# tjuDavidWang/MARL-UAVs-Targets-Tracking

Measured on AMD Instinct MI355X. Metric: env agent-steps/sec, higher is better.
Workload: dtype f32

## Files before the change

### marl-uavs-targets-tracking_amd/csrc/greedy.h

```cpp
#pragma once
#include "env.h"
#include "philox.h"

namespace uavtrack {

template <typename UPos>
__device__ __forceinline__ int greedy_near_count(float2 t, int N, float dc2, UPos upos)
{
    int c = 0;
    for (int j = 0; j < N; ++j) {
        const float2 u = upos(j);
        c += (fmaf(u.y - t.y, u.y - t.y, (u.x - t.x) * (u.x - t.x)) < dc2) ? 1 : 0;
    }
    return c;
}

template <typename UPos, typename TPos, typename Near>
__device__ __forceinline__ int greedy_pick(float x, float y, float h, int i, int N, int M, int na, float dc2,
                                           float turn_unit, uint64_t genv, uint32_t step, uint32_t k0, uint32_t k1,
                                           UPos upos, TPos tpos, Near near)
{
    const Philox4 r = philox4x32_10((uint32_t)genv, step, (uint32_t)i, 0x47524459u ^ (uint32_t)(genv >> 32), k0, k1);
    if (u01(r.v[0]) < 0.25f)
        return (int)(((uint64_t)r.v[1] * (uint32_t)na) >> 32);
    int same = 0;
    for (int j = 0; j < N; ++j) {
        const float2 u = upos(j);
        same += (u.x == x && u.y == y) ? 1 : 0;
    }
    float best = -INFINITY, best_dx = 1.0f, best_dy = 0.0f;
    for (int k = 0; k < M; ++k) {
        const float2 t = tpos(k);
        const float dx = t.x - x, dy = t.y - y;
        const float d2 = fmaf(dy, dy, dx * dx);
        const int others = near(k) - (d2 < dc2 ? same : 0);
        const float score = __builtin_amdgcn_rsqf(d2) - 0.8f * (float)others;
        if (score > best) { best = score; best_dx = dx; best_dy = dy; }
    }
    float angle = atan2f(best_dy, best_dx) - h;
    if (u01(r.v[2]) < 0.3f) angle = 0.0f;
    angle -= kTwoPi * floorf((angle + kPi) * (1.0f / kTwoPi));
    int besta = 0;
    float bestd = INFINITY;
    for (int a = 0; a < na; ++a) {
        const float dd = fabsf(angle - (float)(2 * a + 1 - na) * turn_unit);
        if (dd < bestd) { bestd = dd; besta = a; }
    }
    return besta;
}

}
```

### marl-uavs-targets-tracking_amd/csrc/step_kernel.hip

```cpp

#include "actor.h"
#include "greedy.h"
#include "philox.h"

#include <cstdlib>

#define UAVTRACK_UNROLL_U 5
#define UAVTRACK_UNROLL_T 5

namespace uavtrack {

namespace {

typedef float v2f __attribute__((ext_vector_type(2)));

struct Acc {
    float cntU, iwU, sxU, syU, scU, ssU, saU;
    float cntT, iwT, sxT, syT, scT, ssT;
    float trk;
    float dup;
};

constexpr int kLoneActorTiles = 4;
constexpr float kSymMagic = 12582912.0f;
// ... 92 lines not shown

template <typename T>
__device__ __forceinline__ T *at(T *base, unsigned byte_off)
{
    return (T *)((char *)base + byte_off);
}

typedef unsigned v2u_nt __attribute__((ext_vector_type(2)));
template <typename T>
__device__ __forceinline__ void out_store(T *ptr, T v)
{
    __builtin_nontemporal_store(v, ptr);
}
__device__ __forceinline__ void out_store(uint2 *ptr, unsigned a, unsigned b)
{
    const v2u_nt q = {a, b};
    __builtin_nontemporal_store(q, reinterpret_cast<v2u_nt *>(ptr));
}

__device__ __host__ __forceinline__ int obs_stage_f4(int lanes) { return ((lanes + 63) / 64) * 192; }
__device__ __host__ __forceinline__ int pairs_of(int n) { return (n + 1) >> 1; }
constexpr int kCovPairs = 12;
__device__ __host__ __forceinline__ int cov_words(int m) { return (pairs_of(m) + kCovPairs - 1) / kCovPairs; }
__device__ __host__ __forceinline__ int ustride_of(int n)
{
    const int s = pairs_of(n) * 6;
    return (s * 4) % 64 == 0 ? s + 1 : s;
}
__device__ __host__ __forceinline__ int tstride_of(int m)
{
    const int s = pairs_of(m) * 2;
    return (s * 4) % 64 == 0 ? s + 1 : s;
}

__device__ __host__ __forceinline__ int sym_pose_len(int n) { return n + n / 2 + 1; }
__device__ __host__ __forceinline__ int sym_words(int n, bool z3) { return sym_pose_len(n) * (z3 ? 3 : 2) + 2 * n; }

struct UavRow { float x, y, c, s, a, z; };
__device__ __forceinline__ UavRow uav_elem(const float4 *rows, int j)
{
    const float *f = reinterpret_cast<const float *>(rows + (j >> 1) * 6);
    const int b = j & 1;
    return UavRow{f[b], f[2 + b], f[4 + b], f[6 + b], f[8 + b], f[10 + b]};
}
__device__ __forceinline__ void uav_store(float4 *rows, int j, float x, float y, float c, float s, float a, float z)
{
    float *f = reinterpret_cast<float *>(rows + (j >> 1) * 6);
    const int b = j & 1;
    f[b] = x; f[2 + b] = y; f[4 + b] = c; f[6 + b] = s; f[8 + b] = a; f[10 + b] = z;
}

__device__ __host__ constexpr bool act_bias_shape(int n_spec) { return n_spec > 0 && n_spec <= 64; }

template <int N_, int M_, bool Z3, bool NB, int PF, bool SYM = false, bool VC = false, bool NBSEQ = false>
__device__ __forceinline__ void sweep_fast(const StepParams &p, int N, int M, int i,
                                           const float4 *__restrict__ rowNew, const float4 *__restrict__ rowOld,
                                           const float4 *__restrict__ trow, const v2f *__restrict__ tzrow,
                                           unsigned *__restrict__ covw, int covbase,
                                           float xi, float yi, float zi, float ci, float si, float ai,
                                           float xo, float yo, float zo, float co, float so, float ao, Acc &a,
                                           unsigned long long &nbmask, const float4 *const *__restrict__ rsel = nullptr,
                                           const float4 *__restrict__ ubase = nullptr, unsigned copyw = 0)
{
    const v2f xi2 = splat(xi), yi2 = splat(yi), zi2 = splat(zi);
    const v2f nscale = splat(p.le_neg_scale);
    constexpr bool kActBias = act_bias_shape(N_);
    const int NP = pairs_of(N_ > 0 ? N_ : N), MP = pairs_of(M_ > 0 ? M_ : M);
    constexpr int UU = (N_ > 0 && (N_ + 1) / 2 <= 10) ? (N_ + 1) / 2 : UAVTRACK_UNROLL_U;

    v2f sx = splat(0.f), sy = splat(0.f), sc = splat(0.f), ss = splat(0.f), cnt = splat(0.f), trk = splat(0.f);
    v2f cov = splat(0.f);
    constexpr int QM = M_ > 0 ? (M_ + 1) / 2 : 1, QN = N_ > 0 ? (N_ + 1) / 2 : 1;
    constexpr bool kPrefetch = PF > 0 && N_ > 0 && M_ > 0 && QN <= 10 && QM <= 5 && !Z3;
    float4 Q0[QM], Q1[QM], PN0[QN], PM0[QN], PM1[QN];
    v2f PM2[QN];
    auto copy_row = [&](int jp) -> const float4 * {
        if constexpr (N_ > 0 && N_ <= 64)
            return reinterpret_cast<const float4 *>(reinterpret_cast<const char *>(ubase) + __builtin_amdgcn_ubfe(copyw, (unsigned)jp, 1u) * 48u);
        return (2 * jp < i) ? rowNew : rowOld;
    };
    auto fetch_row = [&](int jq) {
        const float4 *rq = rsel ? rsel[jq] : copy_row(jq);
        PN0[jq] = rowNew[jq * 6]; PM0[jq] = rq[jq * 6]; PM1[jq] = rq[jq * 6 + 1];
        PM2[jq] = *reinterpret_cast<const v2f *>(&rq[jq * 6 + 2]);
    };
    if (kPrefetch) {
#pragma unroll
        for (int kp = 0; kp < QM; ++kp) { Q0[kp] = trow[kp * 2]; Q1[kp] = trow[kp * 2 + 1]; }
#pragma unroll
        for (int jq = 0; jq < PF && jq < QN; ++jq) fetch_row(jq);
        __builtin_amdgcn_sched_barrier(0x407);
    }
    auto target_pair = [&](int kp) {
        const float4 q0 = kPrefetch ? Q0[kPrefetch ? kp : 0] : trow[kp * 2], q1 = kPrefetch ? Q1[kPrefetch ? kp : 0] : trow[kp * 2 + 1];
        const v2f dx = (v2f){q0.x, q0.y} - xi2, dy = (v2f){q0.z, q0.w} - yi2;
        v2f d2 = pk_fma(dy, dy, dx * dx);
        if (Z3) { const v2f dz = tzrow[kp] - zi2; d2 = pk_fma(dz, dz, d2); }
        const v2f dist = {fast_sqrt(d2.x), fast_sqrt(d2.y)};
        const v2f mm = pk_le_mask<VC>(d2, nscale, p.le_dp2);
        sx = pk_fma(mm, dx, sx);
        sy = pk_fma(mm, dy, sy);
        sc = pk_fma(mm, (v2f){q1.x, q1.y}, sc);
        ss = pk_fma(mm, (v2f){q1.z, q1.w}, ss);
        cnt += mm;
        trk = pk_fma(mm, dist, trk);
        cov = pk_fma(cov, splat(4.0f), pk_le_mask<VC>(d2, nscale, p.lt_dp2));
    };
    auto flush_word = [&](int w) {
        const unsigned bits = (unsigned)cov.x | ((unsigned)cov.y << 1);
        if (bits) atomicOr(&covw[covbase + w], bits);
        cov = splat(0.f);
    };
    if constexpr (M_ > 0) {
        constexpr int MPc = (M_ + 1) / 2, CWc = (MPc + kCovPairs - 1) / kCovPairs;
#pragma unroll
        for (int w = 0; w < CWc; ++w) {
            constexpr int kInner = MPc <= UAVTRACK_UNROLL_T ? MPc : 6;
            const int k1 = (w + 1) * kCovPairs < MPc ? (w + 1) * kCovPairs : MPc;
#pragma unroll kInner
            for (int kp = w * kCovPairs; kp < k1; ++kp) target_pair(kp);
            flush_word(w);
        }
    } else {
        for (int w = 0; w * kCovPairs < MP; ++w) {
            const int k1 = min((w + 1) * kCovPairs, MP);
#pragma unroll 4
            for (int kp = w * kCovPairs; kp < k1; ++kp) target_pair(kp);
            flush_word(w);
        }
    }
    a.cntT = cnt.x + cnt.y; a.iwT = a.cntT;
    a.sxT = sx.x + sx.y; a.syT = sy.x + sy.y; a.trk = fmaf(-(trk.x + trk.y), p.inv_dp, 2.0f * a.cntT);
    a.scT = fmaf(sc.x + sc.y, p.vratio, -ci * a.cntT);
    a.ssT = fmaf(ss.x + ss.y, p.vratio, -si * a.cntT);

    sx = splat(0.f); sy = splat(0.f); sc = splat(0.f); ss = splat(0.f); cnt = splat(0.f);
    v2f sa = splat(0.f), dup = splat(0.f);
    constexpr bool NBF = NB && N_ > 0 && (N_ + 1) / 2 <= kCovPairs;
    v2f nbf = splat(0.f);
    const float4 *ub = ubase;
#pragma unroll UU
    for (int jp = 0; jp < NP; ++jp) {
        const float4 *rp;
        if (rsel && kPrefetch) rp = rsel[kPrefetch ? jp : 0] + jp * 6;
        else if constexpr (N_ > 0 && N_ <= 64) rp = reinterpret_cast<const float4 *>(reinterpret_cast<const char *>(ub) + __builtin_amdgcn_ubfe(copyw, (unsigned)jp, 1u) * 48u);
        else rp = copy_row(jp) + jp * 6;
        ub += 6;
        if (kPrefetch) {
            if (jp + PF < NP) fetch_row(jp + PF);
            __builtin_amdgcn_sched_barrier(0x407);
        }
        const float4 n0 = kPrefetch ? PN0[kPrefetch ? jp : 0] : rowNew[jp * 6];
        const float4 m0 = kPrefetch ? PM0[kPrefetch ? jp : 0] : rp[0], m1 = kPrefetch ? PM1[kPrefetch ? jp : 0] : rp[1];
        const float4 m2 = kPrefetch ? make_float4(PM2[kPrefetch ? jp : 0].x, PM2[kPrefetch ? jp : 0].y, 0.f, 0.f) : rp[2];
        const v2f dxn = (v2f){n0.x, n0.y} - xi2, dyn = (v2f){n0.z, n0.w} - yi2;
        const v2f dxm = (v2f){m0.x, m0.y} - xi2, dym = (v2f){m0.z, m0.w} - yi2;
        v2f d2n = pk_fma(dyn, dyn, dxn * dxn), d2m = pk_fma(dym, dym, dxm * dxm);
        if (Z3) {
            const v2f dzm = (v2f){m2.z, m2.w} - zi2;
            d2m = pk_fma(dzm, dzm, d2m);
            if (!SYM || NB) {
                const float4 n2 = rowNew[jp * 6 + 2];
                const v2f dzn = (v2f){n2.z, n2.w} - zi2;
                d2n = pk_fma(dzn, dzn, d2n);
            }
        }
        if (NBF)
            nbf = pk_fma(nbf, splat(4.0f), pk_le_mask<VC>(NBSEQ ? d2m : d2n, nscale, p.le_dp2));
        else if (NB)
            nbmask |= ((unsigned long long)(d2n.x <= p.dp2 ? 1u : 0u) | (unsigned long long)(d2n.y <= p.dp2 ? 2u : 0u)) << (2 * jp);
        if (!SYM) {
            const v2f w = pk_fma((v2f){fast_sqrt(d2n.x), fast_sqrt(d2n.y)}, splat(-p.exp_k1), splat(p.exp_k0));
            dup = pk_fma(pk_le_mask<VC>(d2n, nscale, p.le_two_dp2), (v2f){fast_exp2(w.x), fast_exp2(w.y)}, dup);
        }
        const v2f mm = pk_le_mask<VC>(d2m, nscale, p.le_dc2);
        sx = pk_fma(mm, dxm, sx);
        sy = pk_fma(mm, dym, sy);
        sc = pk_fma(mm, (v2f){m1.x, m1.y}, sc);
        ss = pk_fma(mm, (v2f){m1.z, m1.w}, ss);
        sa = pk_fma(mm, (v2f){m2.x, m2.y}, sa);
        if (!kActBias) cnt += mm;
    }
    if (NBF) {
        const unsigned w = (unsigned)nbf.y | ((unsigned)nbf.x << 1);
        nbmask = (unsigned long long)(__brev(w) >> (32 - 2 * NP));
    }
    const bool odd = i & 1;
    const float dxs = xo - xi, dys = yo - yi;
    float d2s = dist2(dxs, dys);
    if (Z3) { const float dzs = zo - zi; d2s = fmaf(dzs, dzs, d2s); }
    const float mse = (!odd && d2s <= p.dc2) ? 1.0f : 0.0f;
    a.dup = dup.x + dup.y - fast_exp2(p.exp_k0);
    float cnt_all = cnt.x + cnt.y, sa_all = sa.x + sa.y;
    if (kActBias) {
        cnt_all = floorf(sa_all * p.inv_act_bias);
        sa_all = fmaf(-p.act_bias, cnt_all, sa_all);
    }
    a.cntU = cnt_all - (odd ? 1.0f : mse); a.iwU = a.cntU;
    a.sxU = fmaf(-mse, dxs, sx.x + sx.y);
    a.syU = fmaf(-mse, dys, sy.x + sy.y);
    a.scU = fmaf(-mse, co - ci, fmaf(-ci, cnt_all, sc.x + sc.y));
    a.ssU = fmaf(-mse, so - si, fmaf(-si, cnt_all, ss.x + ss.y));
    a.saU = fmaf(-mse, ao - ai, fmaf(-ai, cnt_all, sa_all));
}

template <int N_, bool Z3, bool VC = false>
__device__ __forceinline__ unsigned sym_dup(const StepParams &p, int N, int i, const float *__restrict__ sx, const float *__restrict__ sy,
                                            const float *__restrict__ sz, unsigned *__restrict__ dacc, float xi, float yi, float zi)
{
    const int n = N_ > 0 ? N_ : N;
    const int KP = (n - 1) / 2;
    const v2f xi2 = splat(xi), yi2 = splat(yi), zi2 = splat(zi), nscale = splat(p.le_neg_scale);
    unsigned own = 0;
    struct P2 { v2f x, y, z; };
    auto load2 = [&](int k) {
        P2 q;
        q.x = (v2f){sx[i + k], sx[i + k + 1]};
        q.y = (v2f){sy[i + k], sy[i + k + 1]};
        q.z = Z3 ? (v2f){sz[i + k], sz[i + k + 1]} : splat(0.f);
        return q;
    };
    auto eval2 = [&](const P2 &q) {
        const v2f dx = q.x - xi2, dy = q.y - yi2;
        v2f d2 = pk_fma(dy, dy, dx * dx);
        if (Z3) { const v2f dz = q.z - zi2; d2 = pk_fma(dz, dz, d2); }
        const v2f w = pk_fma((v2f){fast_sqrt(d2.x), fast_sqrt(d2.y)}, splat(-p.exp_k1), splat(p.sym_k0));
        const v2f g = pk_fma(pk_le_mask<VC>(d2, nscale, p.le_two_dp2), (v2f){fast_exp2(w.x), fast_exp2(w.y)}, splat(kSymMagic));
        return make_uint2(__float_as_uint(g.x), __float_as_uint(g.y));
    };
    constexpr int UK = (N_ > 0 && (N_ - 1) / 2 <= 10) ? 5 : 4;
    const int last = KP + ((n & 1) == 0 ? 1 : 0);
    P2 cur = load2(1);
#pragma unroll UK
    for (int k = 1; k + 1 <= KP; k += 2) {
        P2 nxt = cur;
        if (k + 2 <= last) nxt = load2(k + 2);
        const uint2 q = eval2(cur);
        own += q.x + q.y;
        atomicAdd(&dacc[i + k], q.x);
        atomicAdd(&dacc[i + k + 1], q.y);
        cur = nxt;
    }
    if (KP & 1) {
        const uint2 q = eval2(cur);
        own += q.x;
        atomicAdd(&dacc[i + KP], q.x);
        if ((n & 1) == 0) own += q.y;
    } else if ((n & 1) == 0) {
        const uint2 q = eval2(cur);
        own += q.x;
    }
    return own;
}

template <bool Z3>
__device__ __forceinline__ void sweep_weighted(const StepParams &p, int N, int M, int i,
                                               const float4 *__restrict__ rowNew, const float4 *__restrict__ rowOld,
                                               const float4 *__restrict__ trow, const v2f *__restrict__ tzrow,
                                               unsigned *__restrict__ covw, int covbase,
                                               float xi, float yi, float zi, float ci, float si, float ai, float abias, Acc &a)
{
    a = Acc{0, 0, 0, 0, 0, 0, 0, 0, 0, 0, 0, 0, 0, 0, 0};
    unsigned bits = 0;
#pragma unroll 1
    for (int k = 0; k < M; ++k) {
        const float *f = reinterpret_cast<const float *>(trow + (k >> 1) * 2);
        const int b = k & 1;
        const float dx = f[b] - xi, dy = f[2 + b] - yi, tc = f[4 + b], ts = f[6 + b];
        float d2 = dist2(dx, dy);
        if (Z3) { const float dz = reinterpret_cast<const float *>(tzrow)[k] - zi; d2 = fmaf(dz, dz, d2); }
        const float d = fast_sqrt(d2);
        const bool in = d2 <= p.dp2;
        const float m = in ? 1.0f : 0.0f;
        const float rx = dx * p.inv_dp - xi, ry = dy * p.inv_dp - yi;
        const float iw = in ? 1.0f / fminf(sqrtf(rx * rx + ry * ry), 1.0f) : 0.0f;
        a.scT = fmaf(iw, tc * p.vratio - ci, a.scT);
        a.ssT = fmaf(iw, ts * p.vratio - si, a.ssT);
        a.cntT += m;
        a.iwT += iw;
        a.sxT = fmaf(iw, dx, a.sxT);
        a.syT = fmaf(iw, dy, a.syT);
        a.trk = fmaf(m, fmaf(-d, p.inv_dp, 2.0f), a.trk);
        {
            const int kp = k >> 1, word = kp / kCovPairs, MPw = pairs_of(M);
            const int in_word = min(kCovPairs, MPw - word * kCovPairs);
            bits |= (d2 < p.dp2) ? (1u << (2 * (in_word - 1 - kp % kCovPairs) + (k & 1))) : 0u;
            if ((kp % kCovPairs == kCovPairs - 1 && (k & 1)) || k == M - 1) {
                if (bits) atomicOr(&covw[covbase + word], bits);
                bits = 0;
            }
        }
    }
#pragma unroll 1
    for (int j = 0; j < N; ++j) {
        const bool other = (j != i);
        const UavRow nw = uav_elem(rowNew, j);
        const UavRow mx = uav_elem((j < i) ? rowNew : rowOld, j);
        const float dxn = nw.x - xi, dyn = nw.y - yi, dxm = mx.x - xi, dym = mx.y - yi;
        float d2n = dist2(dxn, dyn), d2m = dist2(dxm, dym);
        if (Z3) {
            const float dzn = nw.z - zi, dzm = mx.z - zi;
            d2n = fmaf(dzn, dzn, d2n);
            d2m = fmaf(dzm, dzm, d2m);
        }
        const float ex = fast_exp2(fmaf(fast_sqrt(d2n), -p.exp_k1, p.exp_k0));
        a.dup += (other && d2n <= p.two_dp2) ? ex : 0.0f;
        const bool inm = other && d2m <= p.dc2;
        const float m = inm ? 1.0f : 0.0f;
        const float rx = dxm * p.inv_dc - xi, ry = dym * p.inv_dc - yi;
        const float iw = inm ? 1.0f / fminf(sqrtf(rx * rx + ry * ry), 1.0f) : 0.0f;
        a.scU = fmaf(iw, mx.c - ci, a.scU);
        a.ssU = fmaf(iw, mx.s - si, a.ssU);
        a.saU = fmaf(iw, (mx.a - abias) - ai, a.saU);
        a.cntU += m;
        a.iwU += iw;
        a.sxU = fmaf(iw, dxm, a.sxU);
        a.syU = fmaf(iw, dym, a.syU);
    }
}

template <int N_, int M_, int MODE, bool Z3, int POLICY, bool ALLOUT = false, bool EXTRAS = false, bool LONE = false>
__global__ void __launch_bounds__(kMaxWorkgroup) rollout_kernel(const StepParams p_in)
{
    constexpr bool kVConst = LONE;
    StepParams p = p_in;
    if (kVConst) {
#define UAVTRACK_V(f) p.f = vreg(p_in.f)
        UAVTRACK_V(inv_dp); UAVTRACK_V(inv_dc); UAVTRACK_V(dp2); UAVTRACK_V(dc2); UAVTRACK_V(dup_k); UAVTRACK_V(sym_dup_k);
        UAVTRACK_V(vratio); UAVTRACK_V(inv_na_total); UAVTRACK_V(exp_k0); UAVTRACK_V(exp_k1); UAVTRACK_V(x_max); UAVTRACK_V(y_max);
        UAVTRACK_V(tt_ceil); UAVTRACK_V(inv_tt_ceil); UAVTRACK_V(alpha); UAVTRACK_V(beta); UAVTRACK_V(gamma);
        UAVTRACK_V(sym_k0); UAVTRACK_V(act_bias); UAVTRACK_V(inv_act_bias);
        UAVTRACK_V(le_neg_scale); UAVTRACK_V(le_dp2); UAVTRACK_V(lt_dp2); UAVTRACK_V(le_dc2); UAVTRACK_V(le_two_dp2);
        UAVTRACK_V(dtv_u); UAVTRACK_V(dtv_t); UAVTRACK_V(turn_unit); UAVTRACK_V(inv_na); UAVTRACK_V(two_dp2); UAVTRACK_V(dp); UAVTRACK_V(coop);
#undef UAVTRACK_V
    }
    constexpr bool GREEDY = POLICY == kPolicyGreedy;
    constexpr bool ACTOR = POLICY == kPolicyActor;
    constexpr bool GIVEN = POLICY == kPolicyGiven;
    extern __shared__ float4 smem4[];
    if (ALLOUT) __builtin_assume(p.obs != nullptr && p.reward != nullptr && p.terms != nullptr && p.covered != nullptr && p.done != nullptr);
    if (POLICY == kPolicyGiven) __builtin_assume(p.actions != nullptr);
    const int N = N_ > 0 ? N_ : p.N;
    const int M = M_ > 0 ? M_ : p.M;
    const int E = p.E;
    const int EN = E * N;
    const int CW = cov_words(M);
    const int MP = pairs_of(M);
    const float abias = act_bias_shape(N_) ? p.act_bias : 0.0f;
    const int tid = threadIdx.x;
    const int nthreads = blockDim.x;
    using NbMask = typename NbMaskOf<N_>::type;
    constexpr int kNbBits = 8 * (int)sizeof(NbMask);

    const int ustride = ustride_of(N), tstride = tstride_of(M);
    float4 *utab = smem4;
    float4 *ttab = utab + E * ustride;
    float4 *ostg = ttab + E * tstride;
    float *fb = reinterpret_cast<float *>(ostg + obs_stage_f4(E * N));
    float *thd = fb;   fb += E * M;
// ... 47 lines not shown
            for (int w = 0; w < CW; ++w) covw[e * CW + w] = covw[E * CW + e * CW + w] = 0;
            if (M & 1) {
                float *f = reinterpret_cast<float *>(tenv + (M >> 1) * 2);
                f[1] = kFar; f[3] = kFar; f[5] = 0.f; f[7] = 0.f;
                if (Z3) tzf[e * MP * 2 + M] = 0.f;
            }
        }
    }
    for (int q = tid; q < envs_here * M; q += nthreads) {
        const int te = q / M, k = q - te * M;
        const size_t gt = (size_t)env0 * M + q;
        const float th = S.th[gt];
        float ts, tc;
        sincos_any(th, &ts, &tc);
        float *f = reinterpret_cast<float *>(ttab + te * tstride + (k >> 1) * 2);
        const int bb = k & 1;
        f[bb] = S.tx[gt]; f[2 + bb] = S.ty[gt]; f[4 + bb] = tc; f[6 + bb] = ts;
        thd[q] = th;
        if (Z3) tzf[te * MP * 2 + k] = S.tz[gt];
    }
    const unsigned g32 = (unsigned)g;
    constexpr bool kObsStage = !LONE;
    constexpr bool kObsEarly = kObsStage && POLICY != kPolicyActor;
    const unsigned ostg_off = (((unsigned)env0 * (unsigned)N + (unsigned)(tid & ~63)) * 3u + (unsigned)(tid & 63)) * 16u;
    unsigned lane_off4 = g32 * 4u, lane_off48 = g32 * (unsigned)(UAVTRACK_OBS_DIM * 4);
    size_t row = 0;
    size_t rowb = 0;
    int act_next = 0;
    int act = 0;
    if (GIVEN && active) act = min(max(*at(p.actions, g32 * 4u), 0), p.na_total - 1);
    ActorRng arng;
    arng.valid = false; arng.block = 0;
    float o[12] = {0, 0, 0, 0, 0, 0, 0, 0, 0, 0, 0, 0};
    if (ACTOR && active) {
        const float4 *ip = reinterpret_cast<const float4 *>(p.obs_in + g * UAVTRACK_OBS_DIM);
        const float4 q0 = ip[0], q1 = ip[1], q2 = ip[2];
        o[0] = q0.x; o[1] = q0.y; o[2] = q0.z; o[3] = q0.w; o[4] = q1.x; o[5] = q1.y;
        o[6] = q1.z; o[7] = q1.w; o[8] = q2.x; o[9] = q2.y; o[10] = q2.z; o[11] = q2.w;
        if (EXTRAS && p.auto_reset == kAutoResetContinued && count == 0) {
            o[0] = o[1] = o[2] = o[3] = o[4] = o[5] = o[6] = o[7] = o[8] = -1.0f;
            o[9] = x * p.inv_dc; o[10] = y * p.inv_dc; o[11] = (float)a_prev * p.inv_na_total;
        }
    }
    float *const own0 = reinterpret_cast<float *>(uenv + (i >> 1) * 6) + (i & 1);
    constexpr bool kRegTargets = LONE || (N_ > 0 && N_ <= 20);
    const bool one_target_per_lane = kRegTargets && E * M <= nthreads;
    const bool my_target = tid < envs_here * M;
    float *tgt = reinterpret_cast<float *>(ttab);
    float ttx = 0, tty = 0, ttc = 1, tts = 0, tth = 0;
    if (my_target) {
        const int te = tid / M, k = tid - te * M;
        tgt = reinterpret_cast<float *>(ttab + te * tstride + (k >> 1) * 2) + (k & 1);
    }
    __syncthreads();
    if (one_target_per_lane && my_target) { ttx = tgt[0]; tty = tgt[2]; ttc = tgt[4]; tts = tgt[6]; tth = thd[tid]; }

    constexpr bool kPoolEmit = MODE == UAVTRACK_REWARD_PMI && N_ > 0 && N_ <= 64 && LONE;
    constexpr bool kPipeEmit = MODE == UAVTRACK_REWARD_PMI && N_ > 0 && N_ <= 64 && !LONE;
    constexpr unsigned kPoolBlock = 64;
    unsigned pool_base = 0, pool_left = 0, pend_size = 0, pend_base_v = 0, real_pairs = 0;
    bool pend = false, pend_got = false;
    unsigned pend_base_s = 0;
    auto pool_dummies = [&](unsigned base, unsigned n) {
        for (unsigned k = (unsigned)tid; k < n; k += (unsigned)nthreads) out_store(p.pairs + base + k, 0xFFFFFFFFu, 0u);
    };
    unsigned pe_base = 0, pe_tg = 0;
    int pe_mine = 0, pe_slot = 0;
    NbMask pe_nball = 0, pe_later = 0;
    auto pmi_reward_slot = [&](bool has_neighbours, float raw_i) {
        return has_neighbours ? raw_i : fminf(fmaxf((1.0f - p.coop) * raw_i, -1.0f), 1.0f);
    };
    auto store_record = [&](unsigned tg, unsigned long long nball, unsigned first) {
        if (N <= 32) out_store(reinterpret_cast<uint2 *>(p.nbrec + (size_t)tg * 2), (unsigned)nball, first);
        else {
            uint32_t *rec = p.nbrec + (size_t)tg * 3;
            rec[0] = (unsigned)nball; rec[1] = (unsigned)(nball >> 32); rec[2] = first;
        }
    };
    auto commit_pairs = [&](unsigned base) {
        const unsigned first = base + (unsigned)pe_slot;
        store_record(pe_tg, pe_nball, first);
        if (pe_mine) {
            uint2 *dst = p.pairs + first;
            NbMask later = pe_later;
            while (later) {
                const int j = mffs(later) - 1;
                later &= later - 1;
                out_store(dst++, pe_tg, pe_tg - (unsigned)i + (unsigned)j);
            }
        }
    };

    auto drop_isolated = [&](auto nball, decltype(nball) later) {
        if (mpop(nball) == 1 && later != 0 &&
            reinterpret_cast<const int *>(rawl)[e * (N + 1) + (mffs(later) - 1)] == 1)
            later = 0;
        return later;
    };

    constexpr int kStepsPerIter = (LONE && MODE == UAVTRACK_REWARD_RAW && POLICY == kPolicyGiven && !EXTRAS) ? 2 : 1;
    constexpr int kSelPairs = (kStepsPerIter == 2 && N_ > 0) ? (N_ + 1) / 2 : 1;
    const float4 *selA[kSelPairs], *selB[kSelPairs];
    if (kStepsPerIter == 2) {
#pragma unroll
        for (int jq = 0; jq < kSelPairs; ++jq) {
            selA[jq] = (2 * jq < i) ? uenv : uenv + 3;
            selB[jq] = (2 * jq < i) ? uenv + 3 : uenv;
        }
    }
    const unsigned oldw = (i + 1) / 2 < 32 ? ~0u << ((i + 1) / 2) : 0u;
    constexpr bool kAgeBalance = kStepsPerIter == 2 && N_ == 20 && M_ == 10;
    constexpr unsigned kHwIdWaveSlot = 4u | 0u << 6 | 3u << 11;
    bool favoured = false;
    if (kAgeBalance) favoured = __builtin_amdgcn_s_getreg(kHwIdWaveSlot) != 0;
    const int favoured_steps = (p.T * 3 / 5) & ~1;
    if (kAgeBalance && favoured) __builtin_amdgcn_s_setprio(3);
    for (int t0 = 0; t0 < p.T; t0 += kStepsPerIter) {
        if (kAgeBalance && favoured && t0 == favoured_steps) __builtin_amdgcn_s_setprio(0);
#pragma unroll
    for (int tpar = 0; tpar < kStepsPerIter; ++tpar) {
        const int t = t0 + tpar;
        if (kStepsPerIter > 1 && t >= p.T) break;
        const unsigned tg_off = (unsigned)t * (unsigned)BN + g32;
        const int cbuf = (t & 1) * E * CW;
        uint32_t pk0 = p.greedy_k0, pk1 = p.greedy_k1;
        if (EXTRAS && !GIVEN && p.auto_reset) {
            const uint64_t key = (((uint64_t)p.greedy_k1 << 32) | (uint64_t)p.greedy_k0) + (uint64_t)(uint32_t)epi;
            pk0 = (uint32_t)key; pk1 = (uint32_t)(key >> 32);
        }

        if (GREEDY) {
            const int pc = pn ^ 1;
            auto upos_of = [&](const float4 *rows, int j) {
                const float *f = reinterpret_cast<const float *>(rows + (j >> 1) * 6);
                return make_float2(f[j & 1], f[2 + (j & 1)]);
            };
            auto tpos_of = [&](const float4 *rows, int k) {
                const float *f = reinterpret_cast<const float *>(rows + (k >> 1) * 2);
                return make_float2(f[k & 1], f[2 + (k & 1)]);
            };
            for (int q = tid; q < envs_here * M; q += nthreads) {
                const int te = q / M, k = q - te * M;
                const float4 *rows = utab + te * ustride + pc * 3;
                ncnt[q] = greedy_near_count(tpos_of(ttab + te * tstride, k), N, p.dc2,
                                            [&](int j) { return upos_of(rows, j); });
            }
            __syncthreads();
            if (active) {
                const float4 *rows = uenv + pc * 3;
                act = greedy_pick(x, y, h, i, N, M, p.na, p.dc2, p.turn_unit, (uint64_t)(p.env_offset + b),
                                  (uint32_t)count, pk0, pk1,
                                  [&](int j) { return upos_of(rows, j); },
                                  [&](int k) { return tpos_of(tenv, k); },
                                  [&](int k) { return ncnt[e * M + k]; });
                if (p.actions_out) out_store(at(p.actions_out + row, g32 * 4u), act);
            }
            __syncthreads();
        }

        if (ACTOR) {
            if constexpr (LONE)
                act = actor_pick<false, actor_tiles(Z3), kLoneActorTiles>(o, p.actor_w, kLoneActorTiles, p.na_total, (uint64_t)(p.env_offset + b),
                                        (uint32_t)count, i, pk0, pk1, p.actor_mode, nullptr, arng);
            else
                act = actor_pick<false, actor_tiles(Z3)>(o, p.actor_w, p.actor_hblocks, p.na_total, (uint64_t)(p.env_offset + b),
                                        (uint32_t)count, i, pk0, pk1, p.actor_mode, nullptr, arng);
            if (active && p.actions_out) out_store(at(p.actions_out + row, g32 * 4u), act);
        }

        auto advance_target = [&](float *f, int q) {
            float tx = f[0], ty = f[2];
            tx = fmaf(p.dtv_t, f[4], tx);
            ty = fmaf(p.dtv_t, f[6], ty);
            f[0] = tx; f[2] = ty;
            bool turned = false;
            float th = 0.0f;
            if (0.0f > ty || ty > p.y_max) {
                th = -thd[q];
                turned = true;
            } else if (tx < 0.0f || tx > p.x_max) {
                th = thd[q];
                th = (th > 0.0f) ? kPi - th : -kPi - th;
                turned = true;
            }
            if (turned) {
                float ns, nc;
                sincos_any(th, &ns, &nc);
                f[4] = nc; f[6] = ns;
                thd[q] = th;
            }
        };
        if (one_target_per_lane) {
            if (my_target) {
                ttx = fmaf(p.dtv_t, ttc, ttx);
                tty = fmaf(p.dtv_t, tts, tty);
                tgt[0] = ttx; tgt[2] = tty;
                bool turned = false;
                float th = 0.0f;
                if (0.0f > tty || tty > p.y_max) {
                    th = -tth;
                    turned = true;
                } else if (ttx < 0.0f || ttx > p.x_max) {
                    th = (tth > 0.0f) ? kPi - tth : -kPi - tth;
                    turned = true;
                }
                if (turned) {
                    sincos_any(th, &tts, &ttc);
                    tgt[4] = ttc; tgt[6] = tts;
                    tth = th;
                }
// ... 6 lines not shown
                advance_target(f, q);
                if (EXTRAS && p.tpos) p.tpos[(rowb + env0) * M + q] = make_float2(f[0], f[2]);
            }
        }

        int a_now = 0;
        float ai = 0;
        const float xo = x, yo = y, zo = z, co = c, so = s, ao = (float)a_prev;
        if (active) {
            a_now = GIVEN ? act : min(max(act, 0), p.na_total - 1);
            int a_turn = a_now, a_climb = 0;
            if (Z3) { a_climb = (int)(((float)a_now + 0.5f) * p.inv_na); a_turn = a_now - a_climb * p.na; }
            float step_xy = p.dtv_u;
            if (Z3) {
                step_xy = p.dtv_u * climb_l[a_climb];
                z = fmaf(p.dtv_u, climb_l[UAVTRACK_MAX_CLIMB + a_climb], z);
            }
            x = fmaf(step_xy, c, x);
            y = fmaf(step_xy, s, y);
            ai = (float)a_now;
            h = wrap_heading(fmaf(fmaf(Z3 ? (float)a_turn : ai, 2.0f, (float)(1 - p.na)), p.turn_unit, h));
            sincos_wrapped(h, &s, &c);
            {
                float *f = own0 + pn * 12;
                f[0] = x; f[2] = y; f[4] = c; f[6] = s; f[8] = ai + abias; f[10] = z;
            }
            if (GIVEN && t + 1 < p.T) act_next = *at(p.actions + row + BN, g32 * 4u);
            if (i == 0)
                for (int w = 0; w < CW; ++w) covw[cbuf + e * CW + w] = 0;
            if (kSym) {
                float *sp = symbase + e * symstride;
                unsigned *dq = reinterpret_cast<unsigned *>(sp + (Z3 ? 3 : 2) * symlen);
                sp[i] = x; sp[symlen + i] = y;
                if (Z3) sp[2 * symlen + i] = z;
                if (2 * i <= N) {
                    sp[N + i] = x; sp[symlen + N + i] = y;
                    if (Z3) sp[2 * symlen + N + i] = z;
                }
                dq[i] = 0; dq[N + i] = 0;
            }
            if (kNbSeq) nbt[e * N + i] = 0;
        }
        UAVTRACK_STEP_BARRIER();

        float tt = 0, bp = 0, dupn = 0, raw = 0;
        const float4 *rowNew = uenv + pn * 3;
        const float4 *rowOld = uenv + (pn ^ 1) * 3;
        const v2f *tzrow = reinterpret_cast<const v2f *>(tzf + e * MP * 2);
        constexpr bool kMask = (MODE != UAVTRACK_REWARD_RAW) && N_ > 0 && N_ <= 64;
        unsigned long long nbmask = 0;
        unsigned sym_own = 0;
        constexpr int kPrefetchRows = (LONE && MODE != UAVTRACK_REWARD_MEAN && POLICY == kPolicyGiven) ? 2 : 0;
        if (active) {
            Acc acc;
            const bool near0 = fmaxf(fabsf(x), fabsf(y)) < 2.5f;
            if (__builtin_expect(near0, 0)) {
                sweep_weighted<Z3>(p, N, M, i, rowNew, rowOld, tenv, tzrow, covw, cbuf + e * CW,
                                   x, y, z, c, s, ai, abias, acc);
                if (kMask)
                    for (int j = 0; j < N; ++j) {
                        const UavRow nw = uav_elem(rowNew, j);
                        float d2 = dist2(nw.x - x, nw.y - y);
                        if (Z3) { const float dz = nw.z - z; d2 = fmaf(dz, dz, d2); }
                        nbmask |= (unsigned long long)(d2 <= p.dp2 ? 1u : 0u) << j;
                    }
            } else {
                sweep_fast<N_, M_, Z3, kMask, kPrefetchRows, kSym, kVConst, kNbSeq>(p, N, M, i, rowNew, rowOld, tenv, tzrow, covw, cbuf + e * CW,
                                              x, y, z, c, s, ai, xo, yo, zo, co, so, ao, acc, nbmask,
                                              kStepsPerIter == 2 ? (tpar == 0 ? selA : selB) : nullptr,
                                              uenv, pn ? ~oldw : oldw);
            }
            if (kNbSeq) {
                const unsigned lower = (unsigned)nbmask & ((1u << i) - 1u);
                for (unsigned m = lower; m; m &= m - 1u) atomicOr(&nbt[e * N + __builtin_ctz(m)], 1u << i);
                __builtin_amdgcn_fence(__ATOMIC_RELEASE, "wavefront");
                __builtin_amdgcn_wave_barrier();
                __builtin_amdgcn_fence(__ATOMIC_ACQUIRE, "wavefront");
                nbmask = lower | *reinterpret_cast<volatile unsigned *>(&nbt[e * N + i]);
            }
            if (kSym) {
                const float *sp = symbase + e * symstride;
                unsigned *dq = const_cast<unsigned *>(reinterpret_cast<const unsigned *>(sp + (Z3 ? 3 : 2) * symlen));
                sym_own = sym_dup<N_, Z3, kVConst>(p, N, i, sp, sp + symlen, sp + 2 * symlen, dq, x, y, z);
            }

            {
                const bool anyU = acc.cntU > 0.0f, anyT = acc.cntT > 0.0f;
                const float rcU = anyU ? fast_rcp(acc.cntU) : 0.0f, rcT = anyT ? fast_rcp(acc.cntT) : 0.0f;
                const float baseU = anyU ? 0.0f : -1.0f, baseT = anyT ? 0.0f : -1.0f;
                o[0] = fmaf(acc.sxU * p.inv_dc, rcU, baseU);
                o[1] = fmaf(acc.syU * p.inv_dc, rcU, baseU);
                o[2] = fmaf(acc.scU, rcU, baseU);
                o[3] = fmaf(acc.ssU, rcU, baseU);
                o[4] = fmaf(acc.saU * p.inv_na_total, rcU, baseU);
                o[5] = fmaf(acc.sxT * p.inv_dp, rcT, baseT);
                o[6] = fmaf(acc.syT * p.inv_dp, rcT, baseT);
                o[7] = fmaf(acc.scT, rcT, baseT);
                o[8] = fmaf(acc.ssT, rcT, baseT);
            }
            o[9] = x * p.inv_dc;
            o[10] = y * p.inv_dc;
            o[11] = ai * p.inv_na_total;
            if (kObsEarly && p.obs) {
                float4 *sp = ostg + (tid >> 6) * 192 + (tid & 63) * 3;
                sp[0] = make_float4(o[0], o[1], o[2], o[3]);
                sp[1] = make_float4(o[4], o[5], o[6], o[7]);
                sp[2] = make_float4(o[8], o[9], o[10], o[11]);
            }

            float d_bdr = fminf(fminf(x, p.x_max - x), fminf(y, p.y_max - y));
            if (Z3) d_bdr = fminf(d_bdr, fminf(z, p.z_max - z));
            bp = __builtin_amdgcn_fmed3f(d_bdr * p.inv_dp, 0.0f, 1.0f) - 1.0f;
            tt = __builtin_amdgcn_fmed3f(acc.trk, 0.0f, p.tt_ceil) * p.inv_tt_ceil;
            if (!kSym) dupn = __builtin_amdgcn_fmed3f(acc.dup * p.dup_k, -1.0f, 0.0f);
            if (!kSym) raw = fmaf(p.gamma, dupn, fmaf(p.beta, bp, p.alpha * tt));
            if (MODE == UAVTRACK_REWARD_MEAN) rawl[e * (N + 1) + i] = raw;
            if (MODE == UAVTRACK_REWARD_PMI && kMask) reinterpret_cast<int *>(rawl)[e * (N + 1) + i] = mpop((NbMask)((NbMask)nbmask & ~((NbMask)1 << i)));
        }
        if (kPipeEmit && tid == 0) {
            unsigned *wg_cnt = covw + 2 * E * CW;
            wg_cnt[0] = 0;
            if (t > 0) wg_cnt[1] = pe_base;
        }
        UAVTRACK_STEP_BARRIER();

        if (kPoolEmit && pend && !pend_got) {
            pend_base_s = (unsigned)__builtin_amdgcn_readfirstlane((int)pend_base_v);
            pend_got = true;
        }

        if (active) {
            if (kSym) {
                const unsigned *dq = reinterpret_cast<const unsigned *>(symbase + e * symstride + (Z3 ? 3 : 2) * symlen);
                const float dsum = (float)(sym_own + dq[i] + dq[N + i] - (unsigned)(N - 1) * 0x4B400000u);
                dupn = __builtin_amdgcn_fmed3f(dsum * p.sym_dup_k, -1.0f, 0.0f);
                raw = fmaf(p.gamma, dupn, fmaf(p.beta, bp, p.alpha * tt));
            }
// ... 228 lines not shown
                }
            }
        }
        if (EXTRAS && p.auto_reset) {
            const bool fire = active && p.horizon > 0 && count >= p.horizon;
            if (active && i == 0) rstw[e] = fire ? (unsigned)(epi + 1) + 1u : 0u;
            if (__syncthreads_or(fire ? 1 : 0)) {
                if (fire) {
                    ++epi;
                    const uint64_t genv = (uint64_t)(p.env_offset + b);
                    const Philox4 r = philox4x32_10((uint32_t)genv, (uint32_t)epi, (uint32_t)i, 0x55415631u ^ (uint32_t)(genv >> 32),
                                                    p.reset_k0, p.reset_k1);
                    x = (float)((double)(i + 1) * p.x_max_d / (double)(N + 1));
                    y = (float)(p.y_max_d / 2.0);
                    if (Z3) z = (float)(p.z_max_d / 2.0);
                    h = fmaf(u01(r.v[0]), kTwoPi, -kPi);
                    a_prev = (int)(((uint64_t)r.v[1] * (uint32_t)p.na_total) >> 32);
                    sincos_any(h, &s, &c);
                    count = 0;
                    uav_store(uenv + pn * 3, i, x, y, c, s, (float)a_prev + abias, z);
                    o[0] = o[1] = o[2] = o[3] = o[4] = o[5] = o[6] = o[7] = o[8] = -1.0f;
                    o[9] = x * p.inv_dc; o[10] = y * p.inv_dc; o[11] = (float)a_prev * p.inv_na_total;
                    arng.valid = false;
                    if (p.start_obs) {
                        float4 *so4 = reinterpret_cast<float4 *>(p.start_obs + (row + g) * UAVTRACK_OBS_DIM);
                        so4[0] = make_float4(o[0], o[1], o[2], o[3]);
                        so4[1] = make_float4(o[4], o[5], o[6], o[7]);
                        so4[2] = make_float4(o[8], o[9], o[10], o[11]);
                    }
                }
                auto reset_target = [&](int q, float &tx, float &ty, float &th, float &tc, float &ts) {
                    const int te = q / M, k = q - te * M;
                    const unsigned ep1 = rstw[te];
                    if (!ep1) return false;
                    const uint64_t genv = (uint64_t)(p.env_offset + env0 + te);
                    const Philox4 r = philox4x32_10((uint32_t)genv, ep1 - 1u, (uint32_t)(N + k), 0x55415631u ^ (uint32_t)(genv >> 32),
                                                    p.reset_k0, p.reset_k1);
                    tx = u01(r.v[0]) * p.x_max;
                    ty = u01(r.v[1]) * p.y_max;
                    th = fmaf(u01(r.v[2]), kTwoPi, -kPi);
                    sincos_any(th, &ts, &tc);
                    float *f = reinterpret_cast<float *>(ttab + te * tstride + (k >> 1) * 2) + (k & 1);
                    f[0] = tx; f[2] = ty; f[4] = tc; f[6] = ts;
                    if (Z3) tzf[te * MP * 2 + k] = u01(r.v[3]) * p.z_max;
                    return true;
                };
                if (one_target_per_lane) {
                    if (my_target) reset_target(tid, ttx, tty, tth, ttc, tts);
                } else {
                    for (int q = tid; q < envs_here * M; q += nthreads) {
                        float tx, ty, th, tc, ts;
                        if (reset_target(q, tx, ty, th, tc, ts)) thd[q] = th;
                    }
                }
            }
        }
        pn ^= 1;
        row += BN;
        rowb += (size_t)p.B;
    }
    }
    if (kPoolEmit) {
        pool_dummies(pool_base, pool_left);
        if (pend) pool_dummies(pend_got ? pend_base_s : (unsigned)__builtin_amdgcn_readfirstlane((int)pend_base_v), pend_size);
    }
    if (MODE == UAVTRACK_REWARD_PMI && tid == 0 && real_pairs && p.pair_total)
        atomicAdd(p.pair_total, (unsigned long long)real_pairs);
    if (kPipeEmit && p.T > 0) {
        unsigned *wg_cnt = covw + 2 * E * CW;
        if (tid == 0) wg_cnt[1] = pe_base;
        __syncthreads();
        if (active) commit_pairs(wg_cnt[1]);
    }
    if (CW == 1 && active && i == 0) {
        const int cov = __popc(cov_pending);
        ecov += cov;
        if (p.covered) out_store(p.covered + (rowb - p.B + b), cov);
    }

    if (active) {
        S.ux[g] = x; S.uy[g] = y; S.uh[g] = h; S.ua[g] = a_prev;
        if (Z3) S.uz[g] = z;
        if (i == 0) {
            S.step_count[b] = count;
            if (EXTRAS) S.episode[b] = epi;
        }
    }
    if (EXTRAS && p.state_copy) {
        const StateBlock C2 = state_view(p.state_copy, p.B, N, M, Z3);
        if (active) {
            C2.ux[g] = x; C2.uy[g] = y; C2.uh[g] = h; C2.ua[g] = a_prev;
            if (Z3) C2.uz[g] = z;
            if (i == 0) { C2.step_count[b] = count; C2.episode[b] = epi; }
        }
        for (int q = tid; q < envs_here * M; q += nthreads) {
            const int te = q / M, k = q - te * M;
            const size_t gt = (size_t)env0 * M + q;
            const float *f = reinterpret_cast<const float *>(ttab + te * tstride + (k >> 1) * 2);
            C2.tx[gt] = f[k & 1]; C2.ty[gt] = f[2 + (k & 1)];
            C2.th[gt] = (one_target_per_lane && q == tid) ? tth : thd[q];
            if (Z3) C2.tz[gt] = tzf[te * MP * 2 + k];
        }
    }
    if (EXTRAS && p.auto_reset && Z3)
        for (int q = tid; q < envs_here * M; q += nthreads) {
            const int te = q / M, k = q - te * M;
// ... 216 lines not shown
```

Measured before the change: 41.55 billion.

## Fuse greedy near-count into observation sweep and window the turn search

When the greedy policy is on, the per-target count of nearby UAVs is now accumulated during the main observation sweep through atomic adds, and is reused by the next step's greedy pick. A separate counting pass runs only after resets or when the flags ask for it. The kernel also tracks whether any two UAVs coincide, so the O(N) same-position loop can be skipped when none do. The nearest-turn search now checks a three-entry window around an estimated index instead of scanning all actions. In exchange it adds atomics, flag state in global memory and extra registers, and the correctness of reusing counts across steps depends on sync ordering.

```diff
diff --git a/marl-uavs-targets-tracking_amd/csrc/greedy.h b/marl-uavs-targets-tracking_amd/csrc/greedy.h
--- a/marl-uavs-targets-tracking_amd/csrc/greedy.h
+++ b/marl-uavs-targets-tracking_amd/csrc/greedy.h
@@ -1,5 +1,6 @@
 #pragma once
 #include "env.h"
+#include "greedy_turn.h"
 #include "philox.h"
 
 namespace uavtrack {
@@ -18,15 +19,18 @@
 template <typename UPos, typename TPos, typename Near>
 __device__ __forceinline__ int greedy_pick(float x, float y, float h, int i, int N, int M, int na, float dc2,
                                            float turn_unit, uint64_t genv, uint32_t step, uint32_t k0, uint32_t k1,
-                                           UPos upos, TPos tpos, Near near)
+                                           UPos upos, TPos tpos, Near near, bool count_same = true)
 {
     const Philox4 r = philox4x32_10((uint32_t)genv, step, (uint32_t)i, 0x47524459u ^ (uint32_t)(genv >> 32), k0, k1);
     if (u01(r.v[0]) < 0.25f)
         return (int)(((uint64_t)r.v[1] * (uint32_t)na) >> 32);
-    int same = 0;
-    for (int j = 0; j < N; ++j) {
-        const float2 u = upos(j);
-        same += (u.x == x && u.y == y) ? 1 : 0;
+    int same = 1;
+    if (count_same) {
+        same = 0;
+        for (int j = 0; j < N; ++j) {
+            const float2 u = upos(j);
+            same += (u.x == x && u.y == y) ? 1 : 0;
+        }
     }
     float best = -INFINITY, best_dx = 1.0f, best_dy = 0.0f;
     for (int k = 0; k < M; ++k) {
@@ -40,13 +44,7 @@
     float angle = atan2f(best_dy, best_dx) - h;
     if (u01(r.v[2]) < 0.3f) angle = 0.0f;
     angle -= kTwoPi * floorf((angle + kPi) * (1.0f / kTwoPi));
-    int besta = 0;
-    float bestd = INFINITY;
-    for (int a = 0; a < na; ++a) {
-        const float dd = fabsf(angle - (float)(2 * a + 1 - na) * turn_unit);
-        if (dd < bestd) { bestd = dd; besta = a; }
-    }
-    return besta;
+    return greedy_turn_index(angle, na, turn_unit);
 }
 
 }
diff --git a/marl-uavs-targets-tracking_amd/csrc/greedy_turn.h b/marl-uavs-targets-tracking_amd/csrc/greedy_turn.h
--- /dev/null
+++ b/marl-uavs-targets-tracking_amd/csrc/greedy_turn.h
@@ -0,0 +1,53 @@
+#pragma once
+#include <math.h>
+
+#if defined(__HIPCC__) || defined(__CUDACC__)
+#define UAVTRACK_HD __host__ __device__ inline __attribute__((always_inline))
+#else
+#define UAVTRACK_HD inline
+#endif
+
+namespace uavtrack {
+
+UAVTRACK_HD int greedy_turn_range(float angle, int na, float u, int lo, int hi)
+{
+    int besta = 0;
+    float bestd = INFINITY;
+    for (int a = lo; a <= hi; ++a) {
+        const float dd = fabsf(angle - (float)(2 * a + 1 - na) * u);
+        if (dd < bestd) { bestd = dd; besta = a; }
+    }
+    return besta;
+}
+
+UAVTRACK_HD int greedy_turn_full(float angle, int na, float u) { return greedy_turn_range(angle, na, u, 0, na - 1); }
+
+UAVTRACK_HD bool greedy_turn_windowed_ok(float angle, int na, float u)
+{
+    const float span = (float)na * u;
+    return fabsf(angle) <= 8.0f && span < 3.0e38f && u * 262144.0f >= fmaxf(8.0f, span);
+}
+
+UAVTRACK_HD int greedy_turn_window(float angle, int na, float u, float t)
+{
+    const int a0 = (int)fminf(fmaxf(rintf(t), 0.0f), (float)(na - 1));
+    return greedy_turn_range(angle, na, u, a0 > 0 ? a0 - 1 : 0, a0 + 1 < na ? a0 + 1 : na - 1);
+}
+
+UAVTRACK_HD float greedy_turn_estimate(float angle, int na, float u)
+{
+#if defined(__HIP_DEVICE_COMPILE__)
+    const float q = angle * __builtin_amdgcn_rcpf(u);
+#else
+    const float q = angle / u;
+#endif
+    return (q + (float)(na - 1)) * 0.5f;
+}
+
+UAVTRACK_HD int greedy_turn_index(float angle, int na, float u)
+{
+    if (!greedy_turn_windowed_ok(angle, na, u)) return greedy_turn_full(angle, na, u);
+    return greedy_turn_window(angle, na, u, greedy_turn_estimate(angle, na, u));
+}
+
+}
diff --git a/marl-uavs-targets-tracking_amd/csrc/step_kernel.hip b/marl-uavs-targets-tracking_amd/csrc/step_kernel.hip
--- a/marl-uavs-targets-tracking_amd/csrc/step_kernel.hip
+++ b/marl-uavs-targets-tracking_amd/csrc/step_kernel.hip
@@ -168,16 +168,30 @@
 
 __device__ __host__ constexpr bool act_bias_shape(int n_spec) { return n_spec > 0 && n_spec <= 64; }
 
-template <int N_, int M_, bool Z3, bool NB, int PF, bool SYM = false, bool VC = false, bool NBSEQ = false>
+struct NoTap { static constexpr bool kOn = false; };
+struct GreedyTap {
+    static constexpr bool kOn = true;
+    int *near_env;
+    float lt_dc2;
+    float zmin;
+    v2f nearv, zc;
+};
+struct GreedyAcc : Acc { GreedyTap tap; };
+template <bool GREEDY> struct AccOf { using type = Acc; };
+template <> struct AccOf<true> { using type = GreedyAcc; };
+
+template <int N_, int M_, bool Z3, bool NB, int PF, bool SYM, bool VC, bool NBSEQ, typename TAP>
 __device__ __forceinline__ void sweep_fast(const StepParams &p, int N, int M, int i,
                                            const float4 *__restrict__ rowNew, const float4 *__restrict__ rowOld,
                                            const float4 *__restrict__ trow, const v2f *__restrict__ tzrow,
                                            unsigned *__restrict__ covw, int covbase,
                                            float xi, float yi, float zi, float ci, float si, float ai,
                                            float xo, float yo, float zo, float co, float so, float ao, Acc &a,
-                                           unsigned long long &nbmask, const float4 *const *__restrict__ rsel = nullptr,
-                                           const float4 *__restrict__ ubase = nullptr, unsigned copyw = 0)
-{
+                                           unsigned long long &nbmask, const float4 *const *__restrict__ rsel,
+                                           const float4 *__restrict__ ubase, unsigned copyw,
+                                           TAP *tap)
+{
+    constexpr bool NEAR = TAP::kOn;
     const v2f xi2 = splat(xi), yi2 = splat(yi), zi2 = splat(zi);
     const v2f nscale = splat(p.le_neg_scale);
     constexpr bool kActBias = act_bias_shape(N_);
@@ -221,11 +235,21 @@
         cnt += mm;
         trk = pk_fma(mm, dist, trk);
         cov = pk_fma(cov, splat(4.0f), pk_le_mask<VC>(d2, nscale, p.lt_dp2));
+        if constexpr (NEAR) tap->nearv = pk_fma(tap->nearv, splat(4.0f), pk_le_mask<VC>(d2, nscale, tap->lt_dc2));
     };
     auto flush_word = [&](int w) {
         const unsigned bits = (unsigned)cov.x | ((unsigned)cov.y << 1);
         if (bits) atomicOr(&covw[covbase + w], bits);
         cov = splat(0.f);
+    };
+    [[maybe_unused]] auto flush_near = [](auto *tp, int w, int in_word) {
+        unsigned bits = (unsigned)tp->nearv.x | ((unsigned)tp->nearv.y << 1);
+        while (bits) {
+            const int bit = __ffs((int)bits) - 1;
+            bits &= bits - 1;
+            atomicAdd(&tp->near_env[2 * (w * kCovPairs + in_word - 1 - (bit >> 1)) + (bit & 1)], 1);
+        }
+        tp->nearv = splat(0.f);
     };
     if constexpr (M_ > 0) {
         constexpr int MPc = (M_ + 1) / 2, CWc = (MPc + kCovPairs - 1) / kCovPairs;
@@ -236,6 +260,7 @@
 #pragma unroll kInner
             for (int kp = w * kCovPairs; kp < k1; ++kp) target_pair(kp);
             flush_word(w);
+            if constexpr (NEAR) flush_near(tap, w, k1 - w * kCovPairs);
         }
     } else {
         for (int w = 0; w * kCovPairs < MP; ++w) {
@@ -243,6 +268,7 @@
 #pragma unroll 4
             for (int kp = w * kCovPairs; kp < k1; ++kp) target_pair(kp);
             flush_word(w);
+            if constexpr (NEAR) flush_near(tap, w, k1 - w * kCovPairs);
         }
     }
     a.cntT = cnt.x + cnt.y; a.iwT = a.cntT;
@@ -288,6 +314,7 @@
         if (!SYM) {
             const v2f w = pk_fma((v2f){fast_sqrt(d2n.x), fast_sqrt(d2n.y)}, splat(-p.exp_k1), splat(p.exp_k0));
             dup = pk_fma(pk_le_mask<VC>(d2n, nscale, p.le_two_dp2), (v2f){fast_exp2(w.x), fast_exp2(w.y)}, dup);
+            if constexpr (NEAR) tap->zc += pk_le_mask<VC>(d2n, nscale, 2.0f);
         }
         const v2f mm = pk_le_mask<VC>(d2m, nscale, p.le_dc2);
         sx = pk_fma(mm, dxm, sx);
@@ -301,6 +328,7 @@
         const unsigned w = (unsigned)nbf.y | ((unsigned)nbf.x << 1);
         nbmask = (unsigned long long)(__brev(w) >> (32 - 2 * NP));
     }
+    if constexpr (NEAR && !SYM) tap->zmin = (tap->zc.x + tap->zc.y < 2.0f) ? 1.0f : 0.0f;
     const bool odd = i & 1;
     const float dxs = xo - xi, dys = yo - yi;
     float d2s = dist2(dxs, dys);
@@ -320,10 +348,13 @@
     a.saU = fmaf(-mse, ao - ai, fmaf(-ai, cnt_all, sa_all));
 }
 
-template <int N_, bool Z3, bool VC = false>
+template <int N_, bool Z3, bool VC, typename TAP>
 __device__ __forceinline__ unsigned sym_dup(const StepParams &p, int N, int i, const float *__restrict__ sx, const float *__restrict__ sy,
-                                            const float *__restrict__ sz, unsigned *__restrict__ dacc, float xi, float yi, float zi)
-{
+                                            const float *__restrict__ sz, unsigned *__restrict__ dacc, float xi, float yi, float zi,
+                                            TAP *tap)
+{
+    constexpr bool ZMIN = TAP::kOn;
+    if constexpr (ZMIN) tap->zmin = INFINITY;
     const int n = N_ > 0 ? N_ : N;
     const int KP = (n - 1) / 2;
     const v2f xi2 = splat(xi), yi2 = splat(yi), zi2 = splat(zi), nscale = splat(p.le_neg_scale);
@@ -340,6 +371,7 @@
         const v2f dx = q.x - xi2, dy = q.y - yi2;
         v2f d2 = pk_fma(dy, dy, dx * dx);
         if (Z3) { const v2f dz = q.z - zi2; d2 = pk_fma(dz, dz, d2); }
+        if constexpr (ZMIN) tap->zmin = fminf(tap->zmin, fminf(d2.x, d2.y));
         const v2f w = pk_fma((v2f){fast_sqrt(d2.x), fast_sqrt(d2.y)}, splat(-p.exp_k1), splat(p.sym_k0));
         const v2f g = pk_fma(pk_le_mask<VC>(d2, nscale, p.le_two_dp2), (v2f){fast_exp2(w.x), fast_exp2(w.y)}, splat(kSymMagic));
         return make_uint2(__float_as_uint(g.x), __float_as_uint(g.y));
@@ -369,14 +401,17 @@
     return own;
 }
 
-template <bool Z3>
+template <bool Z3, typename TAP>
 __device__ __forceinline__ void sweep_weighted(const StepParams &p, int N, int M, int i,
                                                const float4 *__restrict__ rowNew, const float4 *__restrict__ rowOld,
                                                const float4 *__restrict__ trow, const v2f *__restrict__ tzrow,
                                                unsigned *__restrict__ covw, int covbase,
-                                               float xi, float yi, float zi, float ci, float si, float ai, float abias, Acc &a)
-{
+                                               float xi, float yi, float zi, float ci, float si, float ai, float abias, Acc &a,
+                                               TAP *tap)
+{
+    constexpr bool NEAR = TAP::kOn;
     a = Acc{0, 0, 0, 0, 0, 0, 0, 0, 0, 0, 0, 0, 0, 0, 0};
+    if constexpr (NEAR) tap->zmin = INFINITY;
     unsigned bits = 0;
 #pragma unroll 1
     for (int k = 0; k < M; ++k) {
@@ -386,6 +421,7 @@
         float d2 = dist2(dx, dy);
         if (Z3) { const float dz = reinterpret_cast<const float *>(tzrow)[k] - zi; d2 = fmaf(dz, dz, d2); }
         const float d = fast_sqrt(d2);
+        if constexpr (NEAR) if (d2 < p.dc2) atomicAdd(&tap->near_env[k], 1);
         const bool in = d2 <= p.dp2;
         const float m = in ? 1.0f : 0.0f;
         const float rx = dx * p.inv_dp - xi, ry = dy * p.inv_dp - yi;
@@ -421,6 +457,7 @@
         }
         const float ex = fast_exp2(fmaf(fast_sqrt(d2n), -p.exp_k1, p.exp_k0));
         a.dup += (other && d2n <= p.two_dp2) ? ex : 0.0f;
+        if constexpr (NEAR) if (other) tap->zmin = fminf(tap->zmin, d2n);
         const bool inm = other && d2m <= p.dc2;
         const float m = inm ? 1.0f : 0.0f;
         const float rx = dxm * p.inv_dc - xi, ry = dym * p.inv_dc - yi;
@@ -574,6 +611,7 @@
         const int te = tid / M, k = tid - te * M;
         tgt = reinterpret_cast<float *>(ttab + te * tstride + (k >> 1) * 2) + (k & 1);
     }
+    if constexpr (GREEDY) if (tid == 0) covw[2 * E * CW] = 2u;
     __syncthreads();
     if (one_target_per_lane && my_target) { ttx = tgt[0]; tty = tgt[2]; ttc = tgt[4]; tts = tgt[6]; tth = thd[tid]; }
 
@@ -651,7 +689,7 @@
             pk0 = (uint32_t)key; pk1 = (uint32_t)(key >> 32);
         }
 
-        if (GREEDY) {
+        if constexpr (GREEDY) {
             const int pc = pn ^ 1;
             auto upos_of = [&](const float4 *rows, int j) {
                 const float *f = reinterpret_cast<const float *>(rows + (j >> 1) * 6);
@@ -661,23 +699,39 @@
                 const float *f = reinterpret_cast<const float *>(rows + (k >> 1) * 2);
                 return make_float2(f[k & 1], f[2 + (k & 1)]);
             };
-            for (int q = tid; q < envs_here * M; q += nthreads) {
-                const int te = q / M, k = q - te * M;
-                const float4 *rows = utab + te * ustride + pc * 3;
-                ncnt[q] = greedy_near_count(tpos_of(ttab + te * tstride, k), N, p.dc2,
-                                            [&](int j) { return upos_of(rows, j); });
-            }
-            __syncthreads();
+            unsigned *const coincw = covw + 2 * E * CW;
+            const float lt_dc2 = p.dc2 * -p.le_neg_scale;
+            const unsigned flags = (unsigned)__builtin_amdgcn_readfirstlane((int)*coincw);
+            const bool exact_same = flags != 0u;
+            if (flags & 2u) {
+                const v2f nscale = splat(p.le_neg_scale);
+                for (int q = tid; q < envs_here * M; q += nthreads) {
+                    const int te = q / M, k = q - te * M;
+                    const float4 *rows = utab + te * ustride + pc * 3;
+                    const float2 tp = tpos_of(ttab + te * tstride, k);
+                    const v2f tx2 = splat(tp.x), ty2 = splat(tp.y);
+                    v2f cnt2 = splat(0.f);
+                    for (int jp = 0; jp < pairs_of(N); ++jp) {
+                        const float4 u = rows[jp * 6];
+                        const v2f dx = (v2f){u.x, u.y} - tx2, dy = (v2f){u.z, u.w} - ty2;
+                        cnt2 += pk_le_mask<kVConst>(pk_fma(dy, dy, dx * dx), nscale, lt_dc2);
+                    }
+                    ncnt[q] = (int)(cnt2.x + cnt2.y);
+                }
+                __syncthreads();
+            }
             if (active) {
                 const float4 *rows = uenv + pc * 3;
                 act = greedy_pick(x, y, h, i, N, M, p.na, p.dc2, p.turn_unit, (uint64_t)(p.env_offset + b),
                                   (uint32_t)count, pk0, pk1,
                                   [&](int j) { return upos_of(rows, j); },
                                   [&](int k) { return tpos_of(tenv, k); },
-                                  [&](int k) { return ncnt[e * M + k]; });
+                                  [&](int k) { return ncnt[e * M + k]; }, exact_same);
                 if (p.actions_out) out_store(at(p.actions_out + row, g32 * 4u), act);
             }
             __syncthreads();
+            for (int q = tid; q < envs_here * M; q += nthreads) ncnt[q] = 0;
+            if (tid == 0) *coincw = 0u;
         }
 
         if (ACTOR) {
@@ -790,11 +844,16 @@
         unsigned sym_own = 0;
         constexpr int kPrefetchRows = (LONE && MODE != UAVTRACK_REWARD_MEAN && POLICY == kPolicyGiven) ? 2 : 0;
         if (active) {
-            Acc acc;
+            typename AccOf<GREEDY>::type acc;
             const bool near0 = fmaxf(fabsf(x), fabsf(y)) < 2.5f;
+            if constexpr (GREEDY) acc.tap = GreedyTap{ncnt + e * M, p.dc2 * -p.le_neg_scale, INFINITY, splat(0.f), splat(0.f)};
             if (__builtin_expect(near0, 0)) {
+                if constexpr (GREEDY)
+                    sweep_weighted<Z3>(p, N, M, i, rowNew, rowOld, tenv, tzrow, covw, cbuf + e * CW,
+                                       x, y, z, c, s, ai, abias, acc, &acc.tap);
+                else
                 sweep_weighted<Z3>(p, N, M, i, rowNew, rowOld, tenv, tzrow, covw, cbuf + e * CW,
-                                   x, y, z, c, s, ai, abias, acc);
+                                   x, y, z, c, s, ai, abias, acc, static_cast<NoTap *>(nullptr));
                 if (kMask)
                     for (int j = 0; j < N; ++j) {
                         const UavRow nw = uav_elem(rowNew, j);
@@ -803,10 +862,14 @@
                         nbmask |= (unsigned long long)(d2 <= p.dp2 ? 1u : 0u) << j;
                     }
             } else {
+                if constexpr (GREEDY)
+                    sweep_fast<N_, M_, Z3, kMask, kPrefetchRows, kSym, kVConst, kNbSeq>(p, N, M, i, rowNew, rowOld, tenv, tzrow, covw, cbuf + e * CW,
+                                                  x, y, z, c, s, ai, xo, yo, zo, co, so, ao, acc, nbmask, nullptr, uenv, pn ? ~oldw : oldw, &acc.tap);
+                else
                 sweep_fast<N_, M_, Z3, kMask, kPrefetchRows, kSym, kVConst, kNbSeq>(p, N, M, i, rowNew, rowOld, tenv, tzrow, covw, cbuf + e * CW,
                                               x, y, z, c, s, ai, xo, yo, zo, co, so, ao, acc, nbmask,
                                               kStepsPerIter == 2 ? (tpar == 0 ? selA : selB) : nullptr,
-                                              uenv, pn ? ~oldw : oldw);
+                                              uenv, pn ? ~oldw : oldw, static_cast<NoTap *>(nullptr));
             }
             if (kNbSeq) {
                 const unsigned lower = (unsigned)nbmask & ((1u << i) - 1u);
@@ -819,8 +882,11 @@
             if (kSym) {
                 const float *sp = symbase + e * symstride;
                 unsigned *dq = const_cast<unsigned *>(reinterpret_cast<const unsigned *>(sp + (Z3 ? 3 : 2) * symlen));
-                sym_own = sym_dup<N_, Z3, kVConst>(p, N, i, sp, sp + symlen, sp + 2 * symlen, dq, x, y, z);
-            }
+                if constexpr (GREEDY) sym_own = sym_dup<N_, Z3, kVConst>(p, N, i, sp, sp + symlen, sp + 2 * symlen, dq, x, y, z, &acc.tap);
+                else
+                sym_own = sym_dup<N_, Z3, kVConst>(p, N, i, sp, sp + symlen, sp + 2 * symlen, dq, x, y, z, static_cast<NoTap *>(nullptr));
+            }
+            if constexpr (GREEDY) if (!(acc.tap.zmin > 0.0f)) covw[2 * E * CW] = 1u;
 
             {
                 const bool anyU = acc.cntU > 0.0f, anyT = acc.cntT > 0.0f;
@@ -1155,6 +1221,10 @@
                         float tx, ty, th, tc, ts;
                         if (reset_target(q, tx, ty, th, tc, ts)) thd[q] = th;
                     }
+                }
+                if constexpr (GREEDY) {
+                    if (tid == 0) covw[2 * E * CW] = 2u;
+                    __syncthreads();
                 }
             }
         }
```

Result: slower. 40.47 billion (-2.6%).
